# MichaelMillerCSU/Koopman-online-updated-MPC

Hardware: AMD Instinct MI355X
Metric: MPC steps/s (lift+EDMD-update+QP, N=20, 20-dim lift) (higher is better)
Workload: dtype f64

## Files before the change

koopman-online-updated-mpc_amd/csrc/qp_rl.h:

```cpp
#pragma once
#include "step_body.h"

namespace kmpc {

__device__ __forceinline__ double half_sum(double s) {
  s += dpp_shr(s, 1);
  s += dpp_shr(s, 2);
  s += dpp_shr(s, 4);
  s += dpp_shr(s, 8);
  double rt = 0.0;
  fmac_rowbcast<15, true>(rt, s, 1.0);
  double r0, r1;
  half_gather(rt, r0, r1);
  return r0 + r1;
}
__device__ __forceinline__ void half_sums_u(double s, double& lo, double& hi) {
  s += dpp_shr(s, 1);
  s += dpp_shr(s, 2);
  s += dpp_shr(s, 4);
  s += dpp_shr(s, 8);
  lo = lane_bcast(s, 15) + lane_bcast(s, 31);
  hi = lane_bcast(s, 47) + lane_bcast(s, 63);
}
__device__ __forceinline__ double dpp_shr_keep(double v, int ctrl) {
// ... 195 lines not shown
    while (true) {
      broke = false;
      for (int pass = 0; pass < 2; ++pass) {
        if (rebuild) {
          KCOUNT(++tc_rebuild);
          if (!half) {
            load_h_rows();
#pragma unroll
            for (int j = 0; j < N_; ++j) M[j] *= 2.0;
          }
          rs = 1.0; rsi = 1.0;
          Smask = 0u;
          carried = false;
          rebuild = false;
        }
        if (Smask != Fmask) {
          if (__builtin_popcount(Smask ^ Fmask) > __builtin_popcount(Fmask) + 2) {
            KCOUNT(++tc_rebuild);
              if (!half) {
              load_h_rows();
#pragma unroll
              for (int j = 0; j < N_; ++j) M[j] *= 2.0;
            }
            rs = 1.0; rsi = 1.0;
            Smask = 0u;
            carried = false;
          }
          KCOUNT(tc_sweeps += __builtin_popcount(Smask ^ Fmask));
          rl_sweep_set<N_>(M, rs, rsi, Smask ^ Fmask, Smask, Fmask, broke, pass == 1, t, half);
        }
        if (!broke || pass == 1) break;
        if (!carried) ++refresh;
        rebuild = true;
      }
      Fmask = Smask;
      if (it == 0 && rounds == 0) KTRACE(10);
      isF = own && ((Fmask >> t) & 1u);
      {
        double lo, hi;
        halves_both_q(rs * rl_matvec<N_>(M, isF ? g : 0.0), lo, hi);
        pdir = lo;
        bool stale = false;
        exact = false;
        for (int kr = 0;; ++kr) {
          halves_both_q(rl_matvec<N_>(M, isF ? pdir : 0.0), lo, hi);
          hp = hi;
          const double r = isF ? g + 2.0 * hp : 0.0;
          if ((unsigned)__ballot(!(tabs(r) <= 1e-13 * gs)) == 0u) { exact = true; break; }
          if (kr >= kr_max || !carried) { stale = carried; break; }
          halves_both_q(rs * rl_matvec<N_>(M, r), lo, hi);
          pdir += lo;
          KCOUNT(++tc_pass);
          nref = kr + 1 > nref ? kr + 1 : nref;
        }
        if (stale) {
          went_stale = true;
          rebuild = true;
          continue;
        }
      }
      if (!predict || broke || rounds >= N_) break;
      const double cand = x + pdir;
      const double over = isF ? (cand - ub > lb - cand ? cand - ub : lb - cand) : -1.0;
      const unsigned offenders = (unsigned)__ballot(over > 0.0);
      if (offenders == 0u) break;
      if (rounds == 0 && __builtin_popcount(offenders) > 2) break;
      const double worst = half_max(over);
      const int jl = __ffs((int)(unsigned)__ballot(over == worst)) - 1;
      const double bj = cand > ub ? ub : lb;
      const double delta = lane_bcast(bj - x, jl);
      if (tid == jl) qx_out[jl] = bj;
      if (own) g += 2.0 * sR[t * NS + jl] * delta;
      Fmask &= ~(1u << jl);
      ++rounds;
    }
    if (it == 0) KTRACE(11);

    double alpha = 1.0, xa = x, hxa = 0.0, Ja = J0;
    bool redo = false;
    while (true) {
      double dstep = pdir;
      if (!isF) {
        const double g0 = 2.0 * hx + fi;
        dstep = own ? ((g0 > 0.0 ? lb : (g0 < 0.0 ? ub : x)) - x) : 0.0;
        if (rounds > 0 && own && !inI) dstep = qx_out[t] - x;
      }
      const double xu = x + alpha * dstep;
      xa = own ? tclip(xu, lb, ub) : 0.0;
      const bool plain = alpha == 1.0 && rounds == 0 && (unsigned)__ballot(own && (isF ? xa != xu : xa != x)) == 0u;
      if (plain) {
        hxa = own ? hx + hp : 0.0;
      } else {
        double lo, hi;
        halves_both_q(rl_matvec<N_>(M, xa), lo, hi);
        hxa = own ? hi : 0.0;
      }
      if (plain && exact) {
        Jok = false;
        break;
      }
      if (!Jok) {
        half_sums_u(own ? x * (hx + fi) : 0.0, J0, Jhi);
        Jok = true;
      }
      const double pJa = own ? xa * (hxa + fi) : 0.0;
      if (rounds > 0) {
        half_sums_u(pJa, Ja, Jhi);
        if (!(Ja <= J0)) redo = true;
        break;
      }
      const double pdec = own ? (isF ? alpha * (-g * pdir) : g * (x - xa)) : 0.0;
      double sD;
      half_sums_u(half ? pdec : pJa, Ja, sD);
      const double mag = tabs(J0) > tabs(Ja) ? tabs(J0) : tabs(Ja);
      if ((J0 - Ja >= 1e-4 * sD - Tol<double>::slack() * mag) || alpha < 1e-10) break;
      if (carried) { redo = true; break; }
      alpha *= 0.25;
      KCOUNT(++tc_ls);
      ++ncrawl;
    }
    if (redo) {
      if (carried && rounds == 0) { rebuild = true; continue; }
      nopredict = true;
      ncrawl += 3;
      continue;
    }
    nopredict = false;
    rtot += rounds;
    x = xa;
    hx = hxa;
    if (Jok) J0 = Ja;
    if (it == 0) KTRACE(12);
    ++it;
  }
  KTRACE(13);
#ifdef KMPC_TRACE
  if (tid == 0 && b < 8192) {
    kmpc_trace_buf[b * 32 + 15] = (unsigned long long)(it + rtot);
    kmpc_trace_buf[b * 32 + 22] += (unsigned long long)tc_sweeps;
    kmpc_trace_buf[b * 32 + 23] += (unsigned long long)tc_rebuild;
    kmpc_trace_buf[b * 32 + 24] += (unsigned long long)tc_pass;
    kmpc_trace_buf[b * 32 + 25] += (unsigned long long)it;
    kmpc_trace_buf[b * 32 + 26] += (unsigned long long)(tc_ls + rtot * 1000);
    kmpc_trace_buf[b * 32 + 27] += (unsigned long long)((tc_carried0 ? 1 : 0) + ((it == 1 && tc_sweeps == 0 && tc_rebuild == 0 && rtot == 0) ? 1000 : 0));
    (void)tc_mv;
  }
#endif
  if (status == 2) x = own ? c0 : 0.0;
  if (status == 3) {
    if (own && !half) qx_out[t] = x;
    cs.valid = 0;
    return true;
  }
  if (own && !half) {
    if (O::has_useq(a)) io_st<IOT>(a.Useq, (size_t)t * B + b, x);
    if (O::warm(a)) a.x_warm[(size_t)t * B + b] = x;
  }
  if (tid == 0) {
    const double uout = O::du_mode(a) ? uprev + x : x;
    *u_slot = x;
    if (O::has_u0(sv)) io_st<IOT>(sv.U0, b, uout);
    if (O::has_u_store(a)) a.u_store[b] = uout;
    if (O::has_plant(a)) {
      double x1, x2;
      if (sv.x_next) { x1 = lds_ld(sv.x_next); x2 = lds_ld(sv.x_next + 1); }
      else { x1 = io_ld<IOT>(a.X_rw, b); x2 = io_ld<IOT>(a.X_rw, (size_t)B + b); }
      plant_apply<double>(a.plant, sv.plant_switched, a.plant_h, x1, x2, uout);
      io_st<IOT>(a.X_rw, b, x1);
      io_st<IOT>(a.X_rw, (size_t)B + b, x2);
      if (sv.x_next) { lds_st(sv.x_next, x1); lds_st(sv.x_next + 1, x2); }
    }
    if (sv.x_next) {
      lds_i32* const acc = (lds_i32*)reinterpret_cast<int*>(sv.x_next + 2);
      acc[0] = acc[0] > status ? acc[0] : status;
      acc[1] += it + rtot;
      acc[2] += 8 * (it + rtot - 1) + 5 * nref + (carried ? 3 * __builtin_popcount(cs.smask ^ Smask) : 3 * N_);
    } else {
      if (a.status) a.status[b] = a.accumulate ? (a.status[b] > status ? a.status[b] : status) : status;
      if (a.iters) a.iters[b] = a.accumulate ? a.iters[b] + it + rtot : it + rtot;
    }
  }
  const bool keep = status == 0 && !(carried && (it >= 4 || nref >= 7));
  if (keep && own && !half) {
    double* const trow = sR + t * NS;
    if constexpr ((N_ & 1) == 0) {
      d2_t* t2 = reinterpret_cast<d2_t*>(__builtin_assume_aligned(trow, 16));
#pragma unroll
      for (int j = 0; j < N_ / 2; ++j) { d2_t v; v.x = M[2 * j]; v.y = M[2 * j + 1]; t2[j] = v; }
    } else {
#pragma unroll
      for (int j = 0; j < N_; ++j) trow[j] = M[j];
    }
  }
  cs.valid = keep ? 1 : 0;
  if (carried_at_start) {
    const int ns = went_stale ? (nstale0 < 255 ? nstale0 + 1 : 255) : 0;
    const int age = full_budget ? 0 : probe_age + 1;
    cs.trust = ns | (age << 8);
  }
  cs.smask = Smask;
  cs.umask = (unsigned)__ballot(own && x >= ub - eact);
  KTRACE(14);
  return false;
}

}
```

koopman-online-updated-mpc_amd/csrc/rollout_kernel.hip:

```cpp
#include "step_body.h"
#include "step_v2.h"
#include "dare_device.h"
#ifdef KMPC_ROLLOUT_JIT_TU
#define dbg_env(name) ((const char*)nullptr)
#endif

namespace kmpc {

typedef double d4_t __attribute__((ext_vector_type(4)));
#ifdef KMPC_TRACE
#define LSTAMP(i)                                                                                      \
  do {                                                                                                 \
    if (wv == 0 && lane == 0 && b0 < 8192) kmpc_lift_buf[(b0 >> 4) * 16 + (i)] = wall_clock64();      \
  } while (0)
__device__ unsigned long long kmpc_lift_buf[512 * 16];
extern "C" int kmpc_lift_trace_read(void* host, size_t bytes) {
  return (int)hipMemcpyFromSymbol(host, HIP_SYMBOL(kmpc_lift_buf), bytes, 0, hipMemcpyDeviceToHost);
}
__device__ unsigned kmpc_step_buf[4096 * 96];
extern "C" int kmpc_step_trace_read(void* host, size_t bytes) {
  return (int)hipMemcpyFromSymbol(host, HIP_SYMBOL(kmpc_step_buf), bytes, 0, hipMemcpyDeviceToHost);
}
#else
#define LSTAMP(i)
// ... 260 lines not shown
        for (int t = 0; t < NT; ++t) {
          const double bv = (t ? v1 : v0) ? bias[16 * (t ? t1 : t0) + drow] : 0.0;
#pragma unroll
          for (int cg = 0; cg < CG; ++cg) { acc[t][cg][0] = bv; acc[t][cg][1] = 0.0; }
        }
        constexpr int NB = 32 / RO_KB2;
#pragma unroll
        for (int g = 0; g < NT * NB; ++g) {
          const int tl = g / NB, kb = (g % NB) * RO_KB2;
          if (g + 1 < NT * NB) {
            const int tl2 = (g + 1) / NB, kb2 = ((g + 1) % NB) * RO_KB2;
            if ((tl2 ? v1 : v0) && kb2 < KS) ro_load_afrags(Wp, KS, tl2 ? t1 : t0, kb2, lane, af[(g + 1) & 1]);
          }
          if ((tl ? v1 : v0) && kb < KS) {
#pragma unroll
            for (int i = 0; i < RO_KB2; ++i)
              if (kb + i < KS) {
#pragma unroll
                for (int cg = 0; cg < CG; ++cg)
                  acc[tl][cg][i & 1] = __builtin_amdgcn_mfma_f64_4x4x4f64(af[g & 1][i], act[(kb + i) * 4 * NC + boff + 4 * cg],
                                                                         acc[tl][cg][i & 1], 0, 0, 0);
              }
          }
        }
#pragma unroll
        for (int t = 0; t < NT; ++t) {
          if (t ? v1 : v0) {
            const int tt = t ? t1 : t0;
#pragma unroll
            for (int cg = 0; cg < CG; ++cg) {
              const double v = acc[t][cg][0] + acc[t][cg][1];
              if (last) sPsi[(16 * tt + drow) * NC + cg * 4 + dcol] = v;
              else actn[(16 * tt + drow) * NC + cg * 4 + dcol] = v > 0.0 ? v : 0.0;
            }
          }
        }
        if (!last) {
          if (h + 1 < R.nhh) { if (vh0) ro_load_afrags(R.Whp[h + 1], KS, th0, 0, lane, af[0]); }
          else if (vo0) ro_load_afrags(R.Wop, KS, to0, 0, lane, af[0]);
        }
        __syncthreads();
      }
      if ((lane & PSI_MASK) < L) psi_i = sPsi[(lane & PSI_MASK) * NC + wv];
    } else {
      const int KS = KS_ > 0 ? KS_ : R.KS, Hp = KS_ > 0 ? (KS_ <= 28 ? 112 : 128) : R.Hp, MTH = Hp >> 4, MTO = R.Lp >> 4;
      const bool hid = wv < MTH, out = wv < MTO;
      if (V2 && !hid && !out) {
        __syncthreads();
        if constexpr (V2) {
          if (live && k > 0 && !RO_NO_UPDATE) {
            int woff0 = (O::D ? h_wbase : R.wbase) + wv * (O::D ? h_wstride : R.wstride), bk0 = b;
            asm volatile("" : "+s"(woff0), "+s"(bk0));
            double* const wsm0 = smem + woff0;
            double uk;
            if constexpr (O::D) uk = u_carry;
            else uk = a.u_prev[bk0];
            const int t0 = lane & 31;
            const double z0 = t0 < L_ ? psi_prev_reg : (t0 == L_ ? uk : 0.0);
            const double gains0 = v2_rls_cov<L_, true>(R.img + (size_t)bk0 * R.img_stride, z0, O::lam(a));
            if (lane < 32 || t0 < L_) v2_cov_slot<N_>(wsm0)[v2_cov_index<L_>(lane)] = gains0;
          } else {
            __syncthreads();
            __syncthreads();
          }
        }
        for (int i = 0; i < R.nhh; ++i) __syncthreads();
      } else if constexpr (ro_encoder_call<L_, N_, Q_>()) {
        ro_encoder_tiles<KS_, NW>(wv, lane, b0, KS, hid, out, R.nhh, R.W1, R.b1, R.Whp[0], R.Whp[1], R.Wop, R.bh[0], R.bh[1], R.bo, sXn, sAct0, sAct1, sPsi);
      } else {
      constexpr int AR = NW == 8 ? 32 : 64;
      const int bl = NW == 8 ? ((lane >> 4) << 3) + (lane & 7) : lane;
      double af[2][RO_KB2];
      if (R.nhh > 0) { if (hid) ro_load_afrags(R.Whp[0], KS, wv, 0, lane, af[0]); }
      else if (out) ro_load_afrags(R.Wop, KS, wv, 0, lane, af[0]);
      double a1 = 0.0;
      d4_t c1 = {0.0, 0.0, 0.0, 0.0};
      if (hid) {
        a1 = R.W1[4 * (16 * wv + (lane & 15)) + (lane >> 4)];
#pragma unroll
        for (int r = 0; r < 4; ++r) c1[r] = R.b1[16 * wv + (lane >> 4) + 4 * r];
      }
      __syncthreads();
      LSTAMP(0);
      if (hid) {
        c1 = __builtin_amdgcn_mfma_f64_16x16x4f64(a1, sXn[4 * (lane & 15) + (lane >> 4)], c1, 0, 0, 0);
#pragma unroll
        for (int r = 0; r < 4; ++r) {
          const int row = 16 * wv + (lane >> 4) + 4 * r;
          if (NW != 8 || (lane & 15) < 8) sAct0[(row >> 2) * AR + (row & 3) * (AR / 4) + (lane & 15)] = c1[r] > 0.0 ? c1[r] : 0.0;
        }
      }
      LSTAMP(1);
      __syncthreads();
      LSTAMP(2);
      for (int h = 0; h <= R.nhh; ++h) {
        const bool last = h == R.nhh;
        const bool mine = last ? out : hid;
        const double* act = (h & 1) ? sAct1 : sAct0;
        double* actn = (h & 1) ? sAct0 : sAct1;
        const double* Wp = last ? R.Wop : R.Whp[h & 1];
        const double* bias = last ? R.bo : R.bh[h & 1];
        d4_t acc0 = {0.0, 0.0, 0.0, 0.0}, acc1 = {0.0, 0.0, 0.0, 0.0};
        if (mine) {
#pragma unroll
          for (int r = 0; r < 4; ++r) acc0[r] = bias[16 * wv + (lane >> 4) + 4 * r];
        }
        if (mine) {
#pragma unroll
          for (int bt = 0; bt < 32 / RO_KB2; ++bt) {
            const int kb = bt * RO_KB2;
            if (kb + RO_KB2 < KS) ro_load_afrags(Wp, KS, wv, kb + RO_KB2, lane, af[(bt + 1) & 1]);
#pragma unroll
            for (int i = 0; i < RO_KB2; i += 2) {
              if (kb + i < KS) acc0 = __builtin_amdgcn_mfma_f64_16x16x4f64(af[bt & 1][i], act[(kb + i) * AR + bl], acc0, 0, 0, 0);
              if (kb + i + 1 < KS)
                acc1 = __builtin_amdgcn_mfma_f64_16x16x4f64(af[bt & 1][i + 1], act[(kb + i + 1) * AR + bl], acc1, 0, 0, 0);
            }
          }
        }
        if (mine) {
          const int col = lane & 15;
#pragma unroll
          for (int r = 0; r < 4; ++r) {
            const int row = 16 * wv + (lane >> 4) + 4 * r;
            const double v = acc0[r] + acc1[r];
            if (last) sPsi[row * 16 + col] = v;
            else if (NW != 8 || col < 8) actn[(row >> 2) * AR + (row & 3) * (AR / 4) + col] = v > 0.0 ? v : 0.0;
          }
        }
        if (!last) {
          if (h + 1 < R.nhh) { if (hid) ro_load_afrags(R.Whp[h + 1], KS, wv, 0, lane, af[0]); }
          else if (out) ro_load_afrags(R.Wop, KS, wv, 0, lane, af[0]);
        }
        LSTAMP(3 + 2 * h);
        __syncthreads();
        LSTAMP(4 + 2 * h);
      }
      }
      if ((lane & PSI_MASK) < L) psi_i = sPsi[(lane & PSI_MASK) * 16 + wv];
    }

#ifdef KMPC_TRACE
    if (lane == 0 && b < 8192) kmpc_trace_buf[b * 32 + 17] = wall_clock64();
    if (lane == 0 && b < 8192 && k == 0) {
      kmpc_trace_buf[b * 32 + 29] = (unsigned long long)__builtin_amdgcn_s_getreg((3 << 11) | 20) | ((unsigned long long)__builtin_amdgcn_s_getreg((31 << 11) | 4) << 8);
      kmpc_trace_buf[b * 32 + 19] = wall_clock64();
      for (int sl = 22; sl < 29; ++sl) kmpc_trace_buf[b * 32 + sl] = 0ull;
    }
#endif
    if (live) {
      int woff = (O::D ? h_wbase : R.wbase) + wv * (O::D ? h_wstride : R.wstride), bk = b;
      asm volatile("" : "+s"(woff), "+s"(bk));
      double* const wsm = smem + woff;
      double* const psi_now = R.psi[cur];
      if (lane < L) psi_now[(size_t)b * L + lane] = psi_i;
      V2DiagOut dgo{nullptr, nullptr, nullptr};
      if constexpr (DIAG) {
        if (R.Psi_log && lane < L) io_st<IOT>(R.Psi_log, ((size_t)k * L + lane) * B + b, psi_i);
        const size_t kb = (size_t)k * B + b;
        dgo.dA = R.dA_log ? io_at<IOT>(R.dA_log, kb) : nullptr;
        dgo.dB = R.dB_log ? io_at<IOT>(R.dB_log, kb) : nullptr;
        dgo.dC = R.dC_log ? io_at<IOT>(R.dC_log, kb) : nullptr;
      }
      StepVar<double> sv;
      sv.psi_now = psi_now;
      sv.psi_prev = R.psi[cur ^ 1];
      sv.psi_in_regs = 1;
      sv.psi_now_v = psi_i;
      sv.psi_prev_v = psi_prev_reg;
      sv.phases = PH_CONDENSE | PH_QP | ((have_prev && !RO_NO_UPDATE) ? PH_RLS : 0);
      sv.first_update = fresh ? 1 : 0;
      sv.plant_switched = (R.switch_step >= 0 && R.step0 + k >= R.switch_step) ? 1 : 0;
      if constexpr (O::D) sv.U0 = a.U0;
      else sv.U0 = R.U_log ? io_at<IOT>(R.U_log, (size_t)k * B) : a.U0;
      if constexpr (O::D) { sv.u_prev_in_regs = k > 0 ? 1 : 0; sv.u_prev_v = u_carry; }
      sv.x_next = RBF ? nullptr : sXn + wv * 4;
      sv.cov_done = (k > 0 && !RO_NO_UPDATE) ? 1 : 0;
      const bool tile_wave = RBF || NW == 4 || wv < ((KS_ > 0 ? (KS_ <= 28 ? 112 : 128) : R.Hp) >> 4) || wv < (R.Lp >> 4);
      sv.cov_ahead = (k + 1 < R.steps && !RO_NO_UPDATE && tile_wave) ? 1 : 0;
      if constexpr (DIAG) {
        if (!(sv.phases & PH_RLS) && lane == 0) {
          if (dgo.dA) io_st<IOT>(dgo.dA, 0, 0.0);
          if (dgo.dB) io_st<IOT>(dgo.dB, 0, 0.0);
          if (dgo.dC) io_st<IOT>(dgo.dC, 0, 0.0);
        }
      }
      constexpr bool LOWREG = ro_max_threads<L_, N_, Q_, NW, KS_>() == 1024 && N_ > 24;
      if constexpr (TERM) {
        StepVar<double> sv1 = sv, sv2 = sv;
        sv1.phases = sv.phases & PH_RLS;
        sv1.cov_ahead = 0;
        sv2.phases = sv.phases & ~PH_RLS;
        double* imgb = V2 ? R.img + (size_t)bk * R.img_stride : nullptr;
        if (sv1.phases) {
          if constexpr (V2) step_v2<L_, N_, Q_, LOWREG, !LOWREG, IOT, 1, DIAG>(a, sv1, bk, wsm, imgb, &dgo);
          else step_body<double, 64, L_, N_, Q_, LOWREG, !LOWREG || Q_ == L_, ro_one_region<L_, N_, Q_, KS_>()>(a, sv1, bk, wsm);
        }
        __threadfence_block();
        block_sync<64>();
        if (R.term_every > 0 && ((R.term_count0 + k) % R.term_every) == 0) {
          double* const scr = R.term_scratch + (size_t)bk * R.term_scratch_stride;
          double* const Wb = R.term_W + (size_t)bk * Q_ * Q_;
          int itd;
          if constexpr (V2) {
            const V2Dims vd(L_, 2);
            const int cy0 = a.cy0;
            itd = wave_dare(L_, Q_, [&](int i, int j) { return imgb[vd.off1(i, j)]; }, [&](int r, int j) { return imgb[vd.off1(L_ + cy0 + r, j)]; },
                            R.term_Q, R.term_R, R.term_eps, R.term_maxiter, a.Qw, scr, Wb);
          } else {
            const double* const Kb = a.K + (size_t)bk * a.strideK;
            const double* const Cb = a.C + (size_t)bk * a.strideC;
            const int cy0 = a.cy0;
            itd = wave_dare(L_, Q_, [&](int i, int j) { return Kb[i * (L_ + 1) + j]; },
                            [&](int r, int j) { return Q_ == L_ ? (r == j ? 1.0 : 0.0) : Cb[(cy0 + r) * L_ + j]; },
                            R.term_Q, R.term_R, R.term_eps, R.term_maxiter, a.Qw, scr, Wb);
          }
          if (R.term_iters && lane == 0) R.term_iters[bk] = itd;
        }
        if constexpr (V2) step_v2<L_, N_, Q_, LOWREG, !LOWREG, IOT, 2>(a, sv2, bk, wsm, imgb);
        else step_body<double, 64, L_, N_, Q_, LOWREG, !LOWREG || Q_ == L_, ro_one_region<L_, N_, Q_, KS_>()>(a, sv2, bk, wsm);
      } else if constexpr (V2) {
        double* imgb = R.img + (size_t)bk * R.img_stride;
        step_v2<L_, N_, Q_, LOWREG, !LOWREG, IOT, 0, DIAG, OPT>(a, sv, bk, wsm, imgb, &dgo);
        if constexpr (O::D) u_carry = uniform_value(lds_ld(v2_u_slot<L_, N_>(wsm)));
      } else {
        step_body<double, 64, L_, N_, Q_, LOWREG, !LOWREG || Q_ == L_, ro_one_region<L_, N_, Q_, KS_>()>(a, sv, bk, wsm);
      }
      if (!O::D && R.X_log) {
        __threadfence_block();
        if (lane < n) io_st<IOT>(R.X_log, ((size_t)k * n + lane) * B + b, io_ld<IOT>(a.X_rw, (size_t)lane * B + b));
      }
    }
#ifdef KMPC_TRACE
    if (lane == 0 && b < 8192) {
      const unsigned long long t18 = wall_clock64();
      kmpc_trace_buf[b * 32 + 18] = t18;
      const unsigned long long dl = kmpc_trace_buf[b * 32 + 17] - kmpc_trace_buf[b * 32 + 16], db = t18 - kmpc_trace_buf[b * 32 + 17];
      if (b < 4096 && k < 32) {
        kmpc_step_buf[b * 96 + 3 * k] = (unsigned)kmpc_trace_buf[b * 32 + 16];
        kmpc_step_buf[b * 96 + 3 * k + 1] = (unsigned)kmpc_trace_buf[b * 32 + 17];
        kmpc_step_buf[b * 96 + 3 * k + 2] = (unsigned)t18;
      }
      kmpc_trace_buf[b * 32 + 20] = (k == 0 ? 0ull : kmpc_trace_buf[b * 32 + 20]) + dl;
      kmpc_trace_buf[b * 32 + 21] = (k == 0 ? 0ull : kmpc_trace_buf[b * 32 + 21]) + db;
    }
#endif
    if (have_prev) fresh = false;
    have_prev = true;
    cur ^= 1;
    psi_prev_reg = psi_i;
  }
  if (!RBF && live && (tid0 & 63) == 0) {
    const int* const acc = reinterpret_cast<const int*>(sXn + wave * 4 + 2);
    if (ra.s.status) ra.s.status[b] = acc[0];
    if (ra.s.iters) ra.s.iters[b] = acc[1];
    if (ra.work) ra.work[b] = acc[2];
  }
}


#undef RO_NO_UPDATE
static int ro_one_region_r2(int n, int L, int q, int N) { return n * L <= N * q ? 0 : ((n * L + 1) & ~1); }
static size_t ro_step_lds_elems(int n, int L, int q, int N, int* r1, int* r2, bool lds_tableau) {
  if (r1) *r1 = step_region1(L, N);
  if (r2) *r2 = step_region2(n, L, N, lds_tableau);
  return step_lds_elems(n, L, q, N, lds_tableau);
}
static size_t rollout_lds_elems(int n, int L, int q, int N, bool rbf, int waves, int Lp, int* wstride) {
  size_t per_wave = (ro_step_lds_elems(n, L, q, N, nullptr, nullptr, !tableau_saves_lds(N, L)) + 1) & ~(size_t)1;
  if (ro_one_region_rt(L, N, q, rbf))
    per_wave = ((size_t)step_region1(L, N) + ro_one_region_r2(n, L, q, N) + vec_elems_one_region(n, L, q, N) + 1) & ~(size_t)1;
  const bool v2 = step_v2_dims(L, N, q);
  if (v2) per_wave = v2_lds_elems(L, q, N);
  if (wstride) *wstride = (int)per_wave;
  size_t elems = per_wave * waves;
  if (rbf) return elems;
  const size_t scratch = ro_scratch_of(waves);
  if (v2) return scratch + elems + ro_keep(Lp, waves);
  if (elems < scratch) elems = scratch;
  return elems + ro_keep(Lp, waves);
}
#if defined(KMPC_ROLLOUT_JIT_TU)
static int g_rollout_workgroup = 0;
#elif defined(KMPC_ROLLOUT_IO32_TU)
extern int g_rollout_workgroup;
#else
int g_rollout_workgroup = 0;
void set_rollout_workgroup(int trajectories) { g_rollout_workgroup = trajectories; }
#endif
static int rollout_waves(int n, int L, int q, int N, bool rbf, int Lp, int B = 1 << 30) {
  const size_t cap = 160 * 1024 / sizeof(double);
  if (!rbf) {
    static const char* env = dbg_env("KMPC_ROLLOUT_WAVES");
    auto wgs = [&](int w) -> int {
      const size_t e = (rollout_lds_elems(n, L, q, N, false, w, Lp, nullptr) + 63) & ~(size_t)63;
      const int k = (int)(cap / e);
      const int maxw = (N > 24 && !ro_one_region_rt(L, N, q, false) && !step_v2_dims(L, N, q)) ? 8 : 16;
      return k * w > maxw ? maxw / w : k;
    };
    if (g_rollout_workgroup) return wgs(g_rollout_workgroup) > 0 ? g_rollout_workgroup : 0;
    if (env && (atoi(env) == 4 || atoi(env) == 8 || atoi(env) == 16)) return wgs(atoi(env)) > 0 ? atoi(env) : 0;
    static int cus_dev[16] = {};
    int& cus = cus_dev[device_slot()];
    if (!cus) {
      int dev = 0;
      if (hipGetDevice(&dev) != hipSuccess || hipDeviceGetAttribute(&cus, hipDeviceAttributeMultiprocessorCount, dev) != hipSuccess || cus <= 0) cus = 256;
    }
    int best = 0, best_traj = 0;
    for (int w = 16; w >= 8; w >>= 1) {
      const int t = wgs(w) * w;
      if (t > best_traj) { best = w; best_traj = t; }
    }
    if (wgs(4) * 4 >= 2 * best_traj && wgs(4) > 0) { best = 4; best_traj = wgs(4) * 4; }
    if (best == 16 && wgs(8) * 8 >= 16 && (B + 15) / 16 < cus) return 8;
    return best;
  }
  for (int w = ro_rbf_eight(L, N, q) ? 8 : 16; w >= 4; --w)
    if (rollout_lds_elems(n, L, q, N, true, w, Lp, nullptr) <= cap) return w;
  return 0;
}
template <int L_, int N_, int Q_, int NW, int KS_, typename IOT = double, bool TERM = false, bool DIAG = false, int OPT = RO_OPT_GENERIC>
static hipError_t launch_rollout_nw(const RolloutArgs<double>& k, int waves, size_t lds, hipStream_t s) {
  static size_t configured_dev[16] = {};
  size_t& configured = configured_dev[device_slot()];
  if (lds > 64 * 1024 && lds > configured) {
    hipError_t e = hipFuncSetAttribute(reinterpret_cast<const void*>(&rollout_kernel<L_, N_, Q_, NW, KS_, IOT, TERM, DIAG, OPT>),
                                       hipFuncAttributeMaxDynamicSharedMemorySize, (int)lds);
    if (e != hipSuccess) return e;
// ... 179 lines not shown
```

koopman-online-updated-mpc_amd/csrc/step_body.h:

```cpp
#pragma once
#include "kernels.h"
#include "plant_device.h"

#ifdef KMPC_TRACE
__device__ unsigned long long kmpc_trace_buf[8192 * 32];
#define KTRACE(slot)                                                                                      \
  do {                                                                                                    \
    if (tid == 0 && b < 8192) kmpc_trace_buf[b * 32 + (slot)] = wall_clock64();                          \
  } while (0)
extern "C" int kmpc_trace_read(void* host, size_t bytes) {
  return (int)hipMemcpyFromSymbol(host, HIP_SYMBOL(kmpc_trace_buf), bytes, 0, hipMemcpyDeviceToHost);
}
#else
#define KTRACE(slot)
#endif

namespace kmpc {

static constexpr int imax(int a, int b) { return a > b ? a : b; }

static constexpr int vec_elems(int n, int L, int q, int N) {
  const int p = L + 1;
  const int setA = 2 * p + 6 * L + n + 2 * N * q;
  const int setB = 3 * N;
  return imax(setA, setB) + N  + 16 ;
}

static constexpr int vec_elems_one_region(int n, int L, int q, int N) {
  return 5 * L + n + 2 * N * q + N + 16;
}
static constexpr int step_region1(int L, int N) { return (imax(imax((L + 1) * (L + 1), L * L), N * N) + 1) & ~1; }
static constexpr int step_region2(int n, int L, int N, bool lds_tableau = true) {
  return (imax(L * (L + 1) + n * L, lds_tableau ? N * N : 0) + 1) & ~1;
}
static constexpr size_t step_lds_elems(int n, int L, int q, int N, bool lds_tableau = true) {
  return (size_t)step_region1(L, N) + step_region2(n, L, N, lds_tableau) + vec_elems(n, L, q, N);
}

template <int TPB> __device__ __forceinline__ void block_sync() {
  if constexpr (TPB == 64) {
    __builtin_amdgcn_fence(__ATOMIC_RELEASE, "wavefront");
    __builtin_amdgcn_wave_barrier();
    __builtin_amdgcn_fence(__ATOMIC_ACQUIRE, "wavefront");
  } else {
    __syncthreads();
  }
}
template <int TPB> __device__ __forceinline__ void block_sync_lds() {
  if constexpr (TPB == 64) {
    block_sync<TPB>();
  } else {
    asm volatile("s_waitcnt lgkmcnt(0)\n\ts_barrier" ::: "memory");
  }
}
template <int TPB> __device__ __forceinline__ int local_tid() {
  int t = TPB == 64 ? (int)__builtin_amdgcn_mbcnt_hi(~0u, __builtin_amdgcn_mbcnt_lo(~0u, 0u)) : (int)threadIdx.x;
  asm volatile("" : "+v"(t));
  return t;
}

template <typename T> struct StepVar {
  int phases, first_update, plant_switched;
  const T* psi_prev;
  const T* psi_now;
  T* U0;
  T* x_next;
  int psi_in_regs;
  T psi_now_v, psi_prev_v;
  bool h_global = false;
  int cov_done = 0, cov_ahead = 0;
  int u_prev_in_regs = 0;
  T u_prev_v = T(0);
};

enum { RO_OPT_GENERIC = 0, RO_OPT_DEFAULT = 1 };
template <int OPT> struct RoOpt {
  static constexpr bool D = OPT == RO_OPT_DEFAULT;
  typedef StepArgs<double> A;
  static __device__ __forceinline__ double lam(const A& a) { if constexpr (D) return 1.0; else return a.lam; }
  static __device__ __forceinline__ int du_mode(const A& a) { if constexpr (D) return 0; else return a.du_mode; }
  static __device__ __forceinline__ int cy0(const A& a) { if constexpr (D) return 0; else return a.cy0; }
  static __device__ __forceinline__ int c_skip_first(const A& a) { if constexpr (D) return 0; else return a.c_skip_first; }
  static __device__ __forceinline__ int ref_per_traj(const A& a) { if constexpr (D) return 0; else return a.ref_per_traj; }
  static __device__ __forceinline__ bool has_wterm(const A& a) { if constexpr (D) return false; else return a.Wterm != nullptr; }
  static __device__ __forceinline__ bool warm(const A& a) { if constexpr (D) return true; else return a.x_warm != nullptr; }
  static __device__ __forceinline__ bool predict(const A& a) { if constexpr (D) return true; else return (a.qp_predict & 1) != 0; }
  static __device__ __forceinline__ int max_iter(const A& a, int N) { if constexpr (D) return 8 * N + 40; else return a.max_iter; }
  static __device__ __forceinline__ bool has_useq(const A& a) { if constexpr (D) return false; else return a.Useq != nullptr; }
  static __device__ __forceinline__ bool has_u_store(const A& a) { if constexpr (D) return true; else return a.u_store != nullptr; }
  static __device__ __forceinline__ bool has_plant(const A& a) { if constexpr (D) return true; else return a.plant >= 0; }
  template <typename SV> static __device__ __forceinline__ bool has_u0(const SV& sv) { if constexpr (D) return true; else return sv.U0 != nullptr; }
};

template <int TPB, int COUNT, typename F> __device__ __forceinline__ void for_strided(int tid, int count, F&& f) {
  if constexpr (COUNT > 0) {
    constexpr int IT = (COUNT + TPB - 1) / TPB;
#pragma unroll
    for (int i = 0; i < IT; ++i) {
      const int e = tid + i * TPB;
      if ((i + 1) * TPB <= COUNT || e < COUNT) f(e, i);
    }
  } else {
    int i = 0;
    for (int e = tid; e < count; e += TPB, ++i) f(e, i);
  }
}

static constexpr bool tableau_saves_lds(int N, int L) { return N * N > L * (L + 1) + 4 * L; }
template <int TPB, int N_, int L_> constexpr bool step_tableau_in_lds() {
  return !(N_ > 0 && L_ > 0 && ((TPB == 64 && N_ <= 40) || (TPB == 256 && N_ <= 64)) && tableau_saves_lds(N_, L_));
}

template <int TPB, int L_, int N_, int Q_> constexpr bool step_one_region() {
  return TPB == 256 && L_ > 0 && N_ > 0 && Q_ > 0 && Q_ != L_ && Q_ <= 2 && (L_ & 3) == 0 && L_ <= 64 &&
         ((L_ + 1) * (L_ + 1) + TPB - 1) / TPB <= 17;
}

template <typename T> struct Tol;
template <> struct Tol<double> {
  static __device__ __forceinline__ double kkt() { return 1e-9; }
  static __device__ __forceinline__ double tight() { return 1e-12; }
  static __device__ __forceinline__ double act() { return 1e-8; }
  static __device__ __forceinline__ double slack() { return 1e-14; }
};
template <> struct Tol<float> {
  static __device__ __forceinline__ float kkt() { return 2e-5f; }
  static __device__ __forceinline__ float tight() { return 2.4e-7f; }
  static __device__ __forceinline__ float act() { return 1e-5f; }
  static __device__ __forceinline__ float slack() { return 1e-6f; }
};

__device__ __forceinline__ double tfma(double a, double b, double c) { return __builtin_fma(a, b, c); }
__device__ __forceinline__ float tfma(float a, float b, float c) { return __builtin_fmaf(a, b, c); }
__device__ __forceinline__ double tabs(double v) { return __builtin_fabs(v); }
__device__ __forceinline__ float tabs(float v) { return __builtin_fabsf(v); }
typedef __attribute__((address_space(3))) double lds_f64;
typedef __attribute__((address_space(3))) int lds_i32;
typedef __attribute__((address_space(3))) float lds_f32;
__device__ __forceinline__ double lds_ld(const double* p) { return *(const lds_f64*)p; }
__device__ __forceinline__ void lds_st(double* p, double v) { *(lds_f64*)p = v; }
__device__ __forceinline__ float lds_ld(const float* p) { return *(const lds_f32*)p; }
__device__ __forceinline__ void lds_st(float* p, float v) { *(lds_f32*)p = v; }
__device__ __forceinline__ double uniform_value(double v) {
  return __hiloint2double(__builtin_amdgcn_readfirstlane(__double2hiint(v)), __builtin_amdgcn_readfirstlane(__double2loint(v)));
}
__device__ __forceinline__ float uniform_value(float v) { return __int_as_float(__builtin_amdgcn_readfirstlane(__float_as_int(v))); }
template <typename T> __device__ __forceinline__ T tclip(T v, T lo, T hi) { return v < lo ? lo : (v > hi ? hi : v); }
template <typename IOT, typename T> __device__ __forceinline__ T io_ld(const T* base, size_t i) { return (T) reinterpret_cast<const IOT*>(base)[i]; }
template <typename IOT, typename T> __device__ __forceinline__ void io_st(T* base, size_t i, T v) { reinterpret_cast<IOT*>(base)[i] = (IOT)v; }
template <typename IOT, typename T> __device__ __forceinline__ T* io_at(T* base, size_t i) { return reinterpret_cast<T*>(reinterpret_cast<IOT*>(base) + i); }
template <typename IOT, typename T> __device__ __forceinline__ const T* io_at(const T* base, size_t i) { return reinterpret_cast<const T*>(reinterpret_cast<const IOT*>(base) + i); }

template <int LANE, bool NOP>
__device__ __forceinline__ void fmac_rowbcast(double& acc, double vec, double coef) {
  if constexpr (NOP)
    asm volatile("s_nop 1\n\tv_fmac_f64_dpp %0, %1, %2 row_newbcast:%3 row_mask:0xf bank_mask:0xf"
                 : "+v"(acc) : "v"(vec), "v"(coef), "n"(LANE));
  else
    asm volatile("v_fmac_f64_dpp %0, %1, %2 row_newbcast:%3 row_mask:0xf bank_mask:0xf"
                 : "+v"(acc) : "v"(vec), "v"(coef), "n"(LANE));
}
struct RowAsm {
  char s[2048];
  int n;
  constexpr const char* data() const { return s; }
  constexpr size_t size() const { return (size_t)n; }
};
template <int L0, int L1, bool PAD> constexpr RowAsm row_dot_text() {
  RowAsm t{};
  auto put = [&t](const char* p) { while (*p) t.s[t.n++] = *p++; };
  auto num = [&t](int v) { if (v >= 10) t.s[t.n++] = (char)('0' + v / 10); t.s[t.n++] = (char)('0' + v % 10); };
  if (PAD) put("s_nop 1\n\t");
  for (int l = L0; l < L1; ++l) {
    put("v_fmac_f64_dpp %0, %"); num(l < 16 ? 1 : 2); put(", %"); num(3 + l - L0);
    put(" row_newbcast:"); num(l & 15); put(" row_mask:0xf bank_mask:0xf");
    if (l + 1 < L1) put("\n\t");
  }
  return t;
}
template <int L0, int L1, bool PAD, int NCOL>
__device__ __forceinline__ void row_dot_block(double& ac, double v0, double v1, const double (&R)[NCOL]) {
  static_assert(L0 >= 0 && L1 > L0 && L1 - L0 <= 26 && L1 <= NCOL && L1 <= 32, "row_dot_block: columns");
#define KMPC_RC(i) "v"(R[L0 + (i) < L1 ? L0 + (i) : L0])
#define KMPC_RC4(i) KMPC_RC(i), KMPC_RC(i + 1), KMPC_RC(i + 2), KMPC_RC(i + 3)
#define KMPC_DOT(...) asm volatile((row_dot_text<L0, L1, PAD>()) : "+v"(ac) : "v"(v0), "v"(v1), __VA_ARGS__)
  constexpr int K = L1 - L0;
  if constexpr (K <= 4) KMPC_DOT(KMPC_RC4(0));
  else if constexpr (K <= 8) KMPC_DOT(KMPC_RC4(0), KMPC_RC4(4));
  else if constexpr (K <= 12) KMPC_DOT(KMPC_RC4(0), KMPC_RC4(4), KMPC_RC4(8));
  else if constexpr (K <= 16) KMPC_DOT(KMPC_RC4(0), KMPC_RC4(4), KMPC_RC4(8), KMPC_RC4(12));
  else if constexpr (K <= 20) KMPC_DOT(KMPC_RC4(0), KMPC_RC4(4), KMPC_RC4(8), KMPC_RC4(12), KMPC_RC4(16));
  else if constexpr (K <= 24) KMPC_DOT(KMPC_RC4(0), KMPC_RC4(4), KMPC_RC4(8), KMPC_RC4(12), KMPC_RC4(16), KMPC_RC4(20));
  else KMPC_DOT(KMPC_RC4(0), KMPC_RC4(4), KMPC_RC4(8), KMPC_RC4(12), KMPC_RC4(16), KMPC_RC4(20), KMPC_RC(24), KMPC_RC(25));
#undef KMPC_DOT
#undef KMPC_RC4
#undef KMPC_RC
}
template <int CNT, int l = 0, int NCOL>
__device__ __forceinline__ void row_dot_stmts(double& ac, double v0, double v1, const double (&R)[NCOL]) {
  if constexpr (l < CNT) {
    if constexpr (l < 16) fmac_rowbcast<l, l == 0>(ac, v0, R[l]);
    else fmac_rowbcast<l - 16, l == 16>(ac, v1, R[l]);
    row_dot_stmts<CNT, l + 1>(ac, v0, v1, R);
  }
}
template <int CNT, bool BLK = true, int NCOL>
__device__ __forceinline__ void row_dot(double& ac, double v0, double v1, const double (&R)[NCOL]) {
  if constexpr (!BLK) {
    row_dot_stmts<CNT>(ac, v0, v1, R);
  } else if constexpr (CNT <= 26) {
    row_dot_block<0, CNT, true>(ac, v0, v1, R);
  } else {
    row_dot_block<0, 16, true>(ac, v0, v1, R);
    row_dot_block<16, CNT, false>(ac, v0, v1, R);
  }
}
template <int LANE, bool NOP, bool LOWHALF>
__device__ __forceinline__ void fmac_rowbcast_m(double& acc, double vec, double coef) {
  if constexpr (LOWHALF) {
    if constexpr (NOP)
      asm volatile("s_nop 1\n\tv_fmac_f64_dpp %0, %1, %2 row_newbcast:%3 row_mask:0x3 bank_mask:0xf" : "+v"(acc) : "v"(vec), "v"(coef), "n"(LANE));
    else
      asm volatile("v_fmac_f64_dpp %0, %1, %2 row_newbcast:%3 row_mask:0x3 bank_mask:0xf" : "+v"(acc) : "v"(vec), "v"(coef), "n"(LANE));
  } else {
    fmac_rowbcast<LANE, NOP>(acc, vec, coef);
  }
}
template <int CNT, int LOWCOL, int l = 0, int NCOL>
__device__ __forceinline__ void row_upd(double (&R)[NCOL], double v0, double v1, double coef) {
  if constexpr (l < CNT) {
    if constexpr (l == 0) asm volatile("" : : "v"(v1));
    fmac_rowbcast_m<(l & 15), l == 0, l == LOWCOL>(R[l], l < 16 ? v0 : v1, coef);
    row_upd<CNT, LOWCOL, l + 1>(R, v0, v1, coef);
  }
}
template <int L_, int l = 0>
__device__ __forceinline__ void chain_dot(double (&ac)[4], double v0, double v1, const double (&row)[L_]) {
  if constexpr (l < L_) {
    if constexpr (l < 16) fmac_rowbcast<l, l == 0>(ac[l & 3], v0, row[l]);
    else fmac_rowbcast<l - 16, l == 16>(ac[l & 3], v1, row[l]);
    chain_dot<L_, l + 1>(ac, v0, v1, row);
  }
}
__device__ __forceinline__ void half_gather(double a, double& v0, double& v1) {
// ... 2114 lines not shown
```

koopman-online-updated-mpc_amd/csrc/step_v2.h:

```cpp
#pragma once
#include "step_body.h"
#include <type_traits>
#include "qp_rl.h"

namespace kmpc {

static constexpr bool step_v2_dims(int L, int N, int q) { return q != L && q > 0 && q <= 2 && L + 2 <= 32 && N <= 32 && L >= 2; }
static constexpr int v2_region1(int N) { return (N * rl_stride(N) + 1) & ~1; }
static constexpr int v2_cov_elems(int L) { return 32 + ((L + 1) & ~1); }
static constexpr int v2_carry_elems(int L) { return 66 + v2_cov_elems(L); }
static constexpr bool v2_chain_dump(int N) { return N < 30; }
static constexpr int v2_vec_elems(int q, int N) { return 16 + 2 * ((N + 1) & ~1) + (q + 2 * N * q) + imax(2 * N, (N + 1) * q + (v2_chain_dump(N) ? (N + 1) * q + 64 : 0)) + 2; }
static constexpr size_t v2_lds_elems(int L, int q, int N) { return ((size_t)v2_region1(N) + v2_carry_elems(L) + v2_vec_elems(q, N) + 1) & ~(size_t)1; }

template <int CNT, int NCOL, bool BLK = true>
__device__ __forceinline__ void rowdot_one(double& ac, double v0, double v1, const double (&R)[NCOL]) {
  row_dot<CNT, BLK>(ac, v0, v1, R);
}
template <int CNT, int NCOL, int LOWCOL>
__device__ __forceinline__ void rowupd(double (&R)[NCOL], double v0, double v1, double coef) {
  row_upd<CNT, LOWCOL>(R, v0, v1, coef);
}
template <int B, int E, typename F> __device__ __forceinline__ void static_for(F&& f) {
  if constexpr (B < E) {
// ... 82 lines not shown
__device__ __forceinline__ void step_v2(const StepArgs<double>& a, const StepVar<double>& sv, const int b, double* const sm, double* const img,
                                        const V2DiagOut* const dg = nullptr) {
  typedef double d2_t __attribute__((ext_vector_type(2)));
  typedef RoOpt<OPT> O;
  constexpr int P_ = L_ + 1, CP = (L_ + 2) / 2, NC = 2 * CP, NX = 2, S2 = 2 * L_ + 1, S1 = L_ + NX;
  constexpr int N = N_, q = Q_;
  static_assert(step_v2_dims(L_, N_, Q_), "step_v2: dimension set");
  static_assert(N_ <= 32 && L_ + 2 <= 32, "step_v2: one variable / one state row per lane of a 32-lane half");
  const int tid = local_tid<64>();
  const int half = tid >> 5, t = tid & 31;
  const int B = a.B;
  double* const sR = sm;
  double* const sCs = sR + v2_region1(N_);
  double* const sCov = sCs + 66;
  double* const vec = sCs + v2_carry_elems(L_);
  double* const red = vec;
  constexpr int NE = (N_ + 1) & ~1;
  double* const sf = red + 16;
  double* const qxo = sf + NE;
  double* const sEr = qxo + NE + q;
  double* const sG = sEr + 2 * N * q;
  double* const dump = sG + (N + 1) * q;
  double* const qxa = sG;
  double* const qg = qxa + N;

  KTRACE(0);
  double up;
  if (O::D && sv.u_prev_in_regs) up = sv.u_prev_v;
  else up = uniform_value(a.u_prev[b]);
  double xw_pre = 0.0;
  constexpr int REFN = (Q_ * N_ + 63) / 64;
  double refp[REFN];
  if (sv.phases & PH_CONDENSE) {
    const double* refg = io_at<IOT>(a.ref, O::ref_per_traj(a) ? (size_t)b * q * N : 0);
#pragma unroll
    for (int i = 0; i < REFN; ++i) {
      const int e = tid + i * 64, ec = e < q * N ? e : 0, k = ec / q, r = ec - k * q;
      refp[i] = io_ld<IOT>(refg, r * N + k);
    }
  }

  double R1[NC];
  const int slot1 = t < S1 ? t : S1 - 1;
  const d2_t* const im = reinterpret_cast<const d2_t*>(img);
  d2_t* const imw = reinterpret_cast<d2_t*>(img);
  const double psin = sv.psi_now_v;
  if (PART != 2 && (sv.phases & PH_RLS)) {
    const bool fu = sv.first_update != 0;
    if (!fu) {
#pragma unroll
      for (int c = 0; c < CP; ++c) {
        const d2_t v = im[CP * S2 + c * S1 + slot1];
        R1[2 * c] = v.x; R1[2 * c + 1] = v.y;
      }
    } else {
#pragma unroll
      for (int c = 0; c < NC; ++c) R1[c] = 0.0;
    }
    const int xr = t - L_ < 0 ? 0 : (t - L_ < NX ? t - L_ : NX - 1);
    double xn;
    if (sv.x_next) xn = lds_ld(sv.x_next + xr);
    else xn = io_ld<IOT>(a.x_now, (size_t)xr * B + b);
    const double z = t < L_ ? sv.psi_prev_v : (t == L_ ? up : 0.0);
    KTRACE(1);
    const double u2 = sv.cov_done ? sCov[v2_cov_index<L_>(tid)] : v2_rls_cov<L_, false>(img, z, O::lam(a));
    KTRACE(2);
    double zv0, zv1;
    gather_rows<(S1 > P_ ? S1 : P_)>(z, zv0, zv1);
    double acc1 = 0.0;
    rowdot_one<P_, NC>(acc1, zv0, zv1, R1);
    KTRACE(3);
    {
      double gall, hall;
      halves_both(u2, gall, hall);
      double g0, g1, h0, h1;
      gather_rows<(S1 > P_ ? S1 : P_)>(gall, g0, g1);
      gather_rows<(S1 > P_ ? S1 : P_)>(hall, h0, h1);
      const bool isK = t < L_, isC = t >= L_ && t < S1;
      double eK = psin - acc1;
      if (O::lam(a) != 1.0) {
        const double linv = 1.0 / O::lam(a);
        eK = eK * linv + psin * (1.0 - linv);
        const double sc = isK ? linv : 1.0;
#pragma unroll
        for (int c = 0; c < P_; ++c) R1[c] *= sc;
      }
      const double cK = isK ? eK : 0.0;
      const double cC = (isC && !(O::c_skip_first(a) && fu)) ? xn - acc1 : 0.0;
      rowupd<P_, NC, -1>(R1, g0, g1, cK);
      rowupd<L_, NC, -1>(R1, h0, h1, cC);
      if constexpr (DIAG) {
        double s1 = half ? cC * cC : cK * cK;
        double s2 = t < L_ ? (half ? hall * hall : gall * gall) : 0.0;
        s1 += dpp_shr(s1, 1); s2 += dpp_shr(s2, 1);
        s1 += dpp_shr(s1, 2); s2 += dpp_shr(s2, 2);
        s1 += dpp_shr(s1, 4); s2 += dpp_shr(s2, 4);
        s1 += dpp_shr(s1, 8); s2 += dpp_shr(s2, 8);
        const double e2 = lane_bcast(s1, 15) + lane_bcast(s1, 31), ec2 = lane_bcast(s1, 47) + lane_bcast(s1, 63);
        const double g2 = lane_bcast(s2, 15) + lane_bcast(s2, 31), h2 = lane_bcast(s2, 47) + lane_bcast(s2, 63);
        const double gL = lane_bcast(gall, L_);
        const double en = __builtin_sqrt(e2), qn = __builtin_nan("");
        if (tid == 0) {
          if (dg->dA) io_st<IOT>(dg->dA, 0, fu ? qn : en * __builtin_sqrt(g2));
          if (dg->dB) io_st<IOT>(dg->dB, 0, fu ? qn : en * __builtin_fabs(gL));
          if (dg->dC) io_st<IOT>(dg->dC, 0, fu ? qn : __builtin_sqrt(ec2) * __builtin_sqrt(h2));
        }
      }
      if (!half && t < S1) {
#pragma unroll
        for (int c = 0; c < CP; ++c) {
          d2_t v;
          v.x = R1[2 * c]; v.y = R1[2 * c + 1];
          imw[CP * S2 + c * S1 + slot1] = v;
        }
      }
    }
    KTRACE(4);
  } else if (PART != 1) {
#pragma unroll
    for (int c = 0; c < CP; ++c) {
      const d2_t v = im[CP * S2 + c * S1 + slot1];
      R1[2 * c] = v.x; R1[2 * c + 1] = v.y;
    }
  }
  if constexpr (PART == 1) return;

  {
    const bool isA = t < L_;
    double v0, v1;
    gather_rows<S1>(isA ? (half ? psin : R1[L_]) : 0.0, v0, v1);
    const double bs = (O::du_mode(a) && isA) ? R1[L_] * (half ? up : 1.0) : 0.0;
    const int ro = t - L_ - O::cy0(a);
    const bool isO = ro >= 0 && ro < q;
    double* const optr = isO ? (half ? sEr - q + ro : sG + ro) : dump + tid;
    KTRACE(5);
    constexpr int JN = N_;
#pragma unroll
    for (int j = 0; j <= JN; ++j) {
      double acc = bs;
      rowdot_one<L_, NC>(acc, v0, v1, R1);
      if constexpr (v2_chain_dump(N_)) optr[j * q] = acc;
      else if (isO) optr[j * q] = acc;
      if (j < JN) gather_rows<S1>(acc, v0, v1);
    }
    block_sync<64>();
#pragma unroll
    for (int i = 0; i < REFN; ++i) {
      const int e = tid + i * 64;
      if (e < q * N) sEr[e] -= refp[i];
    }
    block_sync<64>();
  }
  KTRACE(6);
  if ((sv.phases & PH_QP) && O::warm(a)) xw_pre = a.x_warm[(size_t)(t < N_ ? t : 0) * a.B + b];
  double M[N_];
  double rs = 1.0, rsi = 1.0;
  QpCarry cs;
  {
    const int* const ci = reinterpret_cast<const int*>(sCs + 64);
    cs.smask = (unsigned)__builtin_amdgcn_readfirstlane(ci[0]);
    cs.valid = __builtin_amdgcn_readfirstlane(ci[1]);
    cs.umask = (unsigned)__builtin_amdgcn_readfirstlane(ci[2]);
    cs.trust = __builtin_amdgcn_readfirstlane(ci[3]);
    if (cs.valid) {
      const double* const trow = sR + (t < N_ ? t : N_ - 1) * rl_stride(N_);
      if constexpr ((N_ & 1) == 0) {
        const d2_t* t2 = reinterpret_cast<const d2_t*>(__builtin_assume_aligned(trow, 16));
#pragma unroll
        for (int j = 0; j < N_ / 2; ++j) { const d2_t v = t2[j]; M[2 * j] = v.x; M[2 * j + 1] = v.y; }
      } else {
#pragma unroll
        for (int j = 0; j < N_; ++j) M[j] = trow[j];
      }
      rs = sCs[t];
      rsi = sCs[32 + t];
    }
    block_sync<64>();
  }
  {
    typedef double dq_t __attribute__((ext_vector_type(Q_ == 2 ? 2 : 1)));
    const int hf = tid >> 5, idx = tid & 31;
    const dq_t* const gq = reinterpret_cast<const dq_t*>(__builtin_assume_aligned(sG, Q_ == 2 ? 16 : 8));
    const dq_t* const wq = reinterpret_cast<const dq_t*>(__builtin_assume_aligned((hf ? sEr : sG) + idx * Q_, Q_ == 2 ? 16 : 8));
    double acc = 0.0;
    constexpr int NS = rl_stride(N_);
    double* const h1 = sR - idx * NS;
    double* const h2 = sR - idx;
    const double Qw = a.Qw, rdiag = idx == 0 ? a.Rw : 0.0;
    constexpr int HCH = 10;
    static_for<0, (N_ + HCH - 1) / HCH>([&](auto CC) {
      constexpr int c0 = decltype(CC)::value * HCH, c1 = c0 + HCH < N_ ? c0 + HCH : N_;
      double hv[HCH];
      static_for<c0, c1>([&](auto TT) {
        constexpr int tt = decltype(TT)::value;
        if constexpr (Q_ == 2) {
          const dq_t u = gq[tt], w = wq[tt];
          acc = tfma(u[0], w[0], acc);
          acc = tfma(u[1], w[1], acc);
        } else {
#pragma unroll
          for (int r = 0; r < Q_; ++r) acc = tfma(sG[tt * Q_ + r], ((hf ? sEr : sG) + idx * Q_)[tt * Q_ + r], acc);
        }
        hv[tt - c0] = Qw * acc + rdiag;
      });
      static_for<c0, c1>([&](auto TT) {
        constexpr int tt = decltype(TT)::value;
        lds_store2_lanes<N_ - tt, (N_ - 1 - tt) * (NS + 1) * 8>(h1, h2, hv[tt - c0]);
      });
    });
    if (hf && idx < N_) sf[idx] = 2.0 * Qw * acc;
  }
  if (O::has_wterm(a)) {
    block_sync<64>();
    const double* const Wt = a.Wterm + (a.wterm_per_traj ? (size_t)b * q * q : (size_t)0);
    for (int e = tid; e < N * N; e += 64) {
      const int aa = e / N, bb = e - aa * N;
      const double* ga = sG + (N - 1 - aa) * q;
      const double* gb = sG + (N - 1 - bb) * q;
      double acc = 0.0;
#pragma unroll 1
      for (int r = 0; r < q; ++r)
#pragma unroll 2
        for (int s2 = 0; s2 < q; ++s2) acc += ga[r] * (0.5 * (Wt[r * q + s2] + Wt[s2 * q + r])) * gb[s2];
      sR[aa * rl_stride(N_) + bb] += acc;
    }
    for (int aa = tid; aa < N; aa += 64) {
      const double* ga = sG + (N - 1 - aa) * q;
      const double* eN = sEr + (N - 1) * q;
      double acc = 0.0;
#pragma unroll 1
      for (int r = 0; r < q; ++r)
#pragma unroll 2
        for (int s2 = 0; s2 < q; ++s2) acc += ga[r] * Wt[r * q + s2] * eN[s2];
      sf[aa] += 2.0 * acc;
    }
  }
  block_sync<64>();
  KTRACE(7);

  if (sv.phases & PH_QP) {
    if (qp_rl<N_, IOT, OPT>(sR, sf, a, sv, b, qxo, red + 15, M, rs, rsi, cs, up, xw_pre)) {
#ifdef KMPC_TRACE
      if (tid == 0 && b < 8192) kmpc_trace_buf[b * 32 + 28] += 1ull;
#endif
      block_sync<64>();
      double* const Hg = a.qp_scratch + (size_t)b * N * N;
      for (int e = tid; e < N * N; e += 64) Hg[e] = sR[(e / N) * rl_stride(N_) + (e % N)];
      __threadfence_block();
      block_sync<64>();
      qp_lds<double, 64, IOT>(Hg, sf, sR, qxo, qxa, qg, red, a, sv, b, N, true);
      block_sync<64>();
      for (int e = tid; e < N * q; e += 64) sEr[N * q + e] = 0.0;
      if (tid == 0) red[15] = qxo[0];
    }
    if (!half) {
      sCs[t] = rs;
      sCs[32 + t] = rsi;
    }
    if (tid == 0) {
      int* const ci = reinterpret_cast<int*>(sCs + 64);
      ci[0] = (int)cs.smask;
      ci[1] = cs.valid;
      ci[2] = (int)cs.umask;
      ci[3] = cs.trust;
    }
    block_sync<64>();
    if (sv.cov_ahead) {
      const double uk = (O::du_mode(a) ? up : 0.0) + red[15];
      const double gains = v2_rls_cov<L_, false>(img, t < L_ ? psin : (t == L_ ? uk : 0.0), O::lam(a));
      if (!half || t < L_) sCov[v2_cov_index<L_>(tid)] = gains;
    }
  }
}

template <int L_, int N_, int Q_> __device__ __forceinline__ void step_v2_init(double* const sm) {
  const int tid = local_tid<64>();
  double* const sCs = sm + v2_region1(N_);
  double* const sEr = sCs + v2_carry_elems(L_) + 16 + 2 * ((N_ + 1) & ~1) + Q_;
  if (tid == 0) {
    int* const ci = reinterpret_cast<int*>(sCs + 64);
    ci[0] = 0;
    ci[1] = 0;
    ci[2] = 0;
    ci[3] = 0;
  }
  for (int e = tid; e < N_ * Q_; e += 64) sEr[N_ * Q_ + e] = 0.0;
}

}
```

Before: 157.0 million.

## Keep per-step warm-start, psi and output state in LDS within rollout launch

Inside the multi-step rollout kernel, the warm-start QP solution is now kept in LDS between steps and read from global memory only on the first step and written only on the last. Stores of psi, U0, u_store and plant state to global memory are likewise limited to the final steps of a launch. This removes per-step global memory round trips from the MPC loop. In exchange, intermediate global state is no longer current mid-launch, and the change relies on sf LDS slots being free across steps.

After: 161.0 million, median of 6. 2.6% higher.

```diff
diff --git a/koopman-online-updated-mpc_amd/csrc/qp_rl.h b/koopman-online-updated-mpc_amd/csrc/qp_rl.h
--- a/koopman-online-updated-mpc_amd/csrc/qp_rl.h
+++ b/koopman-online-updated-mpc_amd/csrc/qp_rl.h
@@ -371,22 +371,30 @@
     cs.valid = 0;
     return true;
   }
+  bool launch_last = true;
+  if constexpr ((O::LB & (O::LB_WARM | O::LB_OUT)) != 0) launch_last = O::launch_last(sv);
+  const bool warm_out = (O::LB & O::LB_WARM) ? launch_last : true, store_out = (O::LB & O::LB_OUT) ? launch_last : true;
   if (own && !half) {
     if (O::has_useq(a)) io_st<IOT>(a.Useq, (size_t)t * B + b, x);
-    if (O::warm(a)) a.x_warm[(size_t)t * B + b] = x;
+    if constexpr ((O::LB & O::LB_WARM) != 0) {
+      lds_st(const_cast<double*>(sf) + t, x);
+      if (warm_out) a.x_warm[(size_t)t * B + b] = x;
+    } else if (O::warm(a)) a.x_warm[(size_t)t * B + b] = x;
   }
   if (tid == 0) {
     const double uout = O::du_mode(a) ? uprev + x : x;
     *u_slot = x;
-    if (O::has_u0(sv)) io_st<IOT>(sv.U0, b, uout);
-    if (O::has_u_store(a)) a.u_store[b] = uout;
+    if (O::has_u0(sv) && store_out) io_st<IOT>(sv.U0, b, uout);
+    if (O::has_u_store(a) && store_out) a.u_store[b] = uout;
     if (O::has_plant(a)) {
       double x1, x2;
       if (sv.x_next) { x1 = lds_ld(sv.x_next); x2 = lds_ld(sv.x_next + 1); }
       else { x1 = io_ld<IOT>(a.X_rw, b); x2 = io_ld<IOT>(a.X_rw, (size_t)B + b); }
       plant_apply<double>(a.plant, sv.plant_switched, a.plant_h, x1, x2, uout);
-      io_st<IOT>(a.X_rw, b, x1);
-      io_st<IOT>(a.X_rw, (size_t)B + b, x2);
+      if (store_out || !sv.x_next) {
+        io_st<IOT>(a.X_rw, b, x1);
+        io_st<IOT>(a.X_rw, (size_t)B + b, x2);
+      }
       if (sv.x_next) { lds_st(sv.x_next, x1); lds_st(sv.x_next + 1, x2); }
     }
     if (sv.x_next) {
diff --git a/koopman-online-updated-mpc_amd/csrc/rollout_kernel.hip b/koopman-online-updated-mpc_amd/csrc/rollout_kernel.hip
--- a/koopman-online-updated-mpc_amd/csrc/rollout_kernel.hip
+++ b/koopman-online-updated-mpc_amd/csrc/rollout_kernel.hip
@@ -436,8 +436,9 @@
       int woff = (O::D ? h_wbase : R.wbase) + wv * (O::D ? h_wstride : R.wstride), bk = b;
       asm volatile("" : "+s"(woff), "+s"(bk));
       double* const wsm = smem + woff;
-      double* const psi_now = R.psi[cur];
-      if (lane < L) psi_now[(size_t)b * L + lane] = psi_i;
+      const bool psi_out = !(O::LB & O::LB_PSI) || RBF || k + 2 >= R.steps;
+      double* const psi_now = psi_out ? R.psi[cur] : nullptr;
+      if (psi_out && lane < L) psi_now[(size_t)b * L + lane] = psi_i;
       V2DiagOut dgo{nullptr, nullptr, nullptr};
       if constexpr (DIAG) {
         if (R.Psi_log && lane < L) io_st<IOT>(R.Psi_log, ((size_t)k * L + lane) * B + b, psi_i);
@@ -458,6 +459,7 @@
       if constexpr (O::D) sv.U0 = a.U0;
       else sv.U0 = R.U_log ? io_at<IOT>(R.U_log, (size_t)k * B) : a.U0;
       if constexpr (O::D) { sv.u_prev_in_regs = k > 0 ? 1 : 0; sv.u_prev_v = u_carry; }
+      if constexpr (O::D) { sv.step_k = k; sv.launch_steps = &R.steps; }
       sv.x_next = RBF ? nullptr : sXn + wv * 4;
       sv.cov_done = (k > 0 && !RO_NO_UPDATE) ? 1 : 0;
       const bool tile_wave = RBF || NW == 4 || wv < ((KS_ > 0 ? (KS_ <= 28 ? 112 : 128) : R.Hp) >> 4) || wv < (R.Lp >> 4);
diff --git a/koopman-online-updated-mpc_amd/csrc/step_body.h b/koopman-online-updated-mpc_amd/csrc/step_body.h
--- a/koopman-online-updated-mpc_amd/csrc/step_body.h
+++ b/koopman-online-updated-mpc_amd/csrc/step_body.h
@@ -71,6 +71,8 @@
   int cov_done = 0, cov_ahead = 0;
   int u_prev_in_regs = 0;
   T u_prev_v = T(0);
+  int step_k = 0;
+  const int __attribute__((address_space(4)))* launch_steps = nullptr;
 };
 
 enum { RO_OPT_GENERIC = 0, RO_OPT_DEFAULT = 1 };
@@ -90,6 +92,17 @@
   static __device__ __forceinline__ bool has_u_store(const A& a) { if constexpr (D) return true; else return a.u_store != nullptr; }
   static __device__ __forceinline__ bool has_plant(const A& a) { if constexpr (D) return true; else return a.plant >= 0; }
   template <typename SV> static __device__ __forceinline__ bool has_u0(const SV& sv) { if constexpr (D) return true; else return sv.U0 != nullptr; }
+  enum { LB_PSI = 1, LB_WARM = 2, LB_OUT = 4 };
+#ifndef KMPC_RO_LB
+#define KMPC_RO_LB 7
+#endif
+  static constexpr int LB = D ? (KMPC_RO_LB) : 0;
+  template <typename SV> static __device__ __forceinline__ bool launch_first(const SV& sv) {
+    int k = sv.step_k; asm volatile("" : "+s"(k)); return k == 0;
+  }
+  template <typename SV> static __device__ __forceinline__ bool launch_last(const SV& sv) {
+    int k = sv.step_k; asm volatile("" : "+s"(k)); return k + 1 >= *sv.launch_steps;
+  }
 };
 
 template <int TPB, int COUNT, typename F> __device__ __forceinline__ void for_strided(int tid, int count, F&& f) {
diff --git a/koopman-online-updated-mpc_amd/csrc/step_v2.h b/koopman-online-updated-mpc_amd/csrc/step_v2.h
--- a/koopman-online-updated-mpc_amd/csrc/step_v2.h
+++ b/koopman-online-updated-mpc_amd/csrc/step_v2.h
@@ -258,7 +258,12 @@
     block_sync<64>();
   }
   KTRACE(6);
-  if ((sv.phases & PH_QP) && O::warm(a)) xw_pre = a.x_warm[(size_t)(t < N_ ? t : 0) * a.B + b];
+  if constexpr ((O::LB & O::LB_WARM) != 0) {
+    if (sv.phases & PH_QP) {
+      if (O::launch_first(sv)) xw_pre = a.x_warm[(size_t)(t < N_ ? t : 0) * a.B + b];
+      else xw_pre = lds_ld(sf + (t < N_ ? t : 0));
+    }
+  } else if ((sv.phases & PH_QP) && O::warm(a)) xw_pre = a.x_warm[(size_t)(t < N_ ? t : 0) * a.B + b];
   double M[N_];
   double rs = 1.0, rsi = 1.0;
   QpCarry cs;
@@ -358,6 +363,7 @@
       block_sync<64>();
       for (int e = tid; e < N * q; e += 64) sEr[N * q + e] = 0.0;
       if (tid == 0) red[15] = qxo[0];
+      if constexpr ((O::LB & O::LB_WARM) != 0) { if (tid < N) lds_st(sf + tid, lds_ld(qxo + tid)); }
     }
     if (!half) {
       sCs[t] = rs;
```
